# leeyevi/MV3D_TF

Measured on AMD Instinct MI355X. Metric: KITTI-shape frames/sec (RPN+3-view ROI-pool+NMS) at 1/2/4/8 MI355X, higher is better.
Workload: dtype f32

## Files before the change

include/mv3d_hip.h:

```cpp
#ifndef MV3D_HIP_H
#define MV3D_HIP_H
#include <stddef.h>
#include <stdint.h>
#ifdef __cplusplus
extern "C" {
#endif

typedef enum {
    MV3D_OK = 0,
    MV3D_ERR_INVALID_ARG = 1,
    MV3D_ERR_WORKSPACE = 2,
    MV3D_ERR_HIP = 3,
    MV3D_ERR_ZERO_DIVISION = 4
} mv3d_status;

int mv3d_version(void);
const char *mv3d_status_string(int status);


size_t mv3d_nms_workspace_bytes(int max_boxes);
int mv3d_nms_device(const float *dets_dev, int n, double thresh, int max_keep,
                    int32_t *keep_dev, int32_t *num_keep_dev, int32_t *status_dev,
                    void *workspace, size_t workspace_bytes, void *stream);

// ... 210 lines not shown
size_t mv3d_point_cloud_2_top_paper_workspace(int num_frames, const double *ranges8_host);
int mv3d_point_cloud_2_top_paper_shape(double res, double zres, double side_lo, double side_hi, double fwd_lo, double fwd_hi,
                                       double height_lo, double height_hi, int *dims);
int mv3d_bev_density_table(float *out64);

size_t mv3d_scan_crop_workspace(int total_points);
int mv3d_scan_crop_tile_rows(void);
int mv3d_scan_crop_to_image(const float *points_dev, const int32_t *offsets_dev, int num_frames, int total_points,
                            const float *calib_dev, const int32_t *image_hw_dev, float *points_out_dev, int32_t *offsets_out_dev,
                            void *workspace_dev, size_t workspace_bytes, void *stream);

int mv3d_scan_transform(const float *points_dev, const int32_t *offsets_dev, int num_frames, int total_points,
                        const double *xform_dev, float *points_out_dev, void *stream);

int mv3d_legacy_permutation(void *mt19937_state, int32_t n, int32_t *out);
typedef struct {
    int32_t n_fg, n_bg, n_low;
    int32_t pt_n_fg, pt_n_bg;
    int32_t reserved0;
    const uint8_t *fg_alive;
} mv3d_draw_frame;
typedef struct {
    int32_t rpn_batchsize;
    int32_t rpn_num_fg;
    int32_t rois_per_image;
    int32_t roi_fg_max;
} mv3d_draw_params;
int mv3d_draw_training_subsamples(void *mt19937_state, int batch, const mv3d_draw_frame *frames, const mv3d_draw_params *par,
                                  int32_t *lists, size_t lists_cap, int32_t *sizes, int32_t *scratch, size_t scratch_cap);

typedef struct {
    int32_t batch, H, W, num_classes;
    int32_t proposal_cap;
    int32_t anchor_cap;
    int32_t roi_cap;
    int32_t max_gt;
    mv3d_proposal_params proposal;
    mv3d_anchor_target_params anchor;
    mv3d_proposal_target_params target;
    mv3d_draw_params draw;
} mv3d_train_path_config;
typedef struct {
    float *blob_bv, *blob_img, *blob_3d;
    int32_t *num_proposals;
// ... 5 lines not shown
    int32_t *pt_counts;
    void *anchor_ws; size_t anchor_ws_bytes;
    void *target_ws; size_t target_ws_bytes;
    float *rois_bev, *rois_rgb, *rois_fv;
    float *rois_3d; int32_t *labels; float *bbox_targets;
    int32_t *lists; size_t lists_cap;
    uint8_t *h_report; size_t h_report_row;
    int32_t *h_pt_counts;
    int32_t *h_num_proposals;
    int32_t *h_lists;
    int32_t *h_scratch; size_t scratch_cap;
} mv3d_train_path_slot;
typedef struct mv3d_train_path mv3d_train_path;
int mv3d_train_path_create(const mv3d_train_path_config *config, int depth, const mv3d_train_path_slot *slots, int helper_thread,
                           mv3d_train_path **out);
int mv3d_train_path_configure(mv3d_train_path *path, const mv3d_train_path_config *config);
int mv3d_train_path_submit(mv3d_train_path *path, int slot, const float *prob_dev, const float *pred_dev, const float *im_info_dev,
                           const float *calib_dev, const float *const *gt_bv_dev, const float *const *gt_3d_dev,
                           const float *const *gt_corners_dev, const int *G, void *mt19937_state, void *stream);
int mv3d_train_path_submit_masked(mv3d_train_path *path, int slot, const float *prob_dev, const float *pred_dev,
                                  const float *im_info_dev, const float *calib_dev, const float *const *gt_bv_dev,
                                  const float *const *gt_3d_dev, const float *const *gt_corners_dev, const int *G,
                                  const uint8_t *anchor_mask_dev, void *mt19937_state, void *stream);
int mv3d_train_path_finish(mv3d_train_path *path, int slot, int32_t *rows_out, int32_t *num_proposals_out, int32_t *sizes_out);
int mv3d_train_path_host_seconds(mv3d_train_path *path, double *wait_s, double *draw_s);
void mv3d_train_path_destroy(mv3d_train_path *path);
int mv3d_train_path_launch_plan(const mv3d_train_path_config *config, int32_t *stage1_launches, int32_t *stage2_launches);

int mv3d_gt_encode(const float *box_cam_dev, const double *cos_sin_dev, int num_objects, const float *inv_rot_dev,
                   const float *tr_velo_to_cam_dev, float *corners_cam_dev, float *corners_lidar_dev,
                   float *boxes_3d_dev, float *boxes_bv_dev, void *stream);

int mv3d_box_detect_tail(const float *rois_3d_dev, const float *bbox_pred_dev, int num_rois, int num_classes,
                         float *corners_dev, float *pred_cnr_r_dev, float *pred_bv_dev, float *pred_bv_r_dev,
                         void *stream);

typedef struct {
    int32_t num_classes;
    int32_t rows_per_frame;
    int32_t max_per_image;
// ... 253 lines not shown
```

mv3d_tf_amd/_lib.py:

```python
import ctypes as C
import os

import torch

_HERE = os.path.dirname(os.path.abspath(__file__))
LIB_PATH = os.path.join(_HERE, "libmv3d_hip.so")

OK, ERR_INVALID_ARG, ERR_WORKSPACE, ERR_HIP, ERR_ZERO_DIVISION = 0, 1, 2, 3, 4
MAX_ROI_VIEWS = 4


class ProposalParams(C.Structure):
    _fields_ = [("feat_stride", C.c_int32), ("pre_nms_topN", C.c_int32), ("post_nms_topN", C.c_int32),
                ("img_height", C.c_int32), ("img_width", C.c_int32), ("img_padding", C.c_int32),
                ("nms_strict_gt", C.c_int32), ("reserved0", C.c_int32), ("nms_thresh", C.c_double), ("min_size", C.c_double)]


class DetectPostParams(C.Structure):
    _fields_ = [("num_classes", C.c_int32), ("rows_per_frame", C.c_int32), ("max_per_image", C.c_int32),
                ("nms_strict_gt", C.c_int32), ("score_thresh", C.c_float), ("reserved0", C.c_int32), ("nms_thresh", C.c_double)]


class AnchorTargetParams(C.Structure):
    _fields_ = [("feat_stride", C.c_int32), ("clobber_positives", C.c_int32),
# ... 189 lines not shown
    "mv3d_roi_pool_backward_workspace_bytes": (C.c_size_t, [C.c_int, C.POINTER(RoiGradView), C.c_int, C.c_int]),
    "mv3d_roi_pool_backward_views": (C.c_int, [C.c_int, C.POINTER(RoiGradView), C.c_int, C.c_int, _P, C.c_size_t, _P]),
    "mv3d_roi_pool_backward_path": (C.c_char_p, [C.c_int, C.POINTER(RoiGradView), C.c_int, C.c_int, C.c_int, C.c_int]),
    "mv3d_roi_pool_pair_workspace_bytes": (C.c_size_t, [C.c_int, C.POINTER(RoiGradView), C.c_int, C.c_int]),
    "mv3d_roi_pool_forward_views_pair": (C.c_int, [C.c_int, C.POINTER(RoiView), C.c_int, C.c_int, C.c_int, _P]),
    "mv3d_roi_pool_backward_views_pair": (C.c_int, [C.c_int, C.POINTER(RoiGradView), C.c_int, C.c_int, _P, C.c_size_t, _P]),
    "mv3d_roi_pool_argmax_decode": (C.c_int, [C.c_int, C.POINTER(RoiView), C.c_int, C.c_int, C.POINTER(C.c_void_p), _P]),
    "mv3d_ROIPoolForwardLaucher": (C.c_int, [_P, C.c_float, C.c_int, C.c_int, C.c_int, C.c_int, C.c_int, C.c_int, _P, _P, _P, _P]),
    "mv3d_ROIPoolBackwardLaucher": (C.c_int, [_P, C.c_float, C.c_int, C.c_int, C.c_int, C.c_int, C.c_int, C.c_int, C.c_int, _P, _P, _P, _P]),
    "mv3d_rois_3d_to_fv": (C.c_int, [_P, C.c_int, _P, _P]),
    "mv3d_point_cloud_2_front_workspace": (C.c_size_t, [C.c_int]),
    "mv3d_point_cloud_2_front": (C.c_int, [_P, _P, C.c_int, C.c_int, _P, _P, _P]),
    "mv3d_legacy_permutation": (C.c_int, [_P, C.c_int32, _P]),
    "mv3d_draw_training_subsamples": (C.c_int, [_P, C.c_int, C.POINTER(DrawFrame), C.POINTER(DrawParams), _P, C.c_size_t, _P, _P,
                                                C.c_size_t]),
    "mv3d_train_path_create": (C.c_int, [C.POINTER(TrainPathConfig), C.c_int, C.POINTER(TrainPathSlot), C.c_int, C.POINTER(C.c_void_p)]),
    "mv3d_train_path_configure": (C.c_int, [_P, C.POINTER(TrainPathConfig)]),
    "mv3d_train_path_submit": (C.c_int, [_P, C.c_int, _P, _P, _P, _P, _P, _P, _P, _P, _P, _P]),
    "mv3d_train_path_submit_masked": (C.c_int, [_P, C.c_int, _P, _P, _P, _P, _P, _P, _P, _P, _P, _P, _P]),
    "mv3d_train_path_finish": (C.c_int, [_P, C.c_int, _P, _P, _P]),
    "mv3d_train_path_host_seconds": (C.c_int, [_P, C.POINTER(C.c_double), C.POINTER(C.c_double)]),
    "mv3d_train_path_destroy": (None, [_P]),
    "mv3d_train_path_launch_plan": (C.c_int, [_P, C.POINTER(C.c_int32), C.POINTER(C.c_int32)]),
    "mv3d_gt_encode": (C.c_int, [_P, _P, C.c_int, _P, _P, _P, _P, _P, _P, _P]),
    "mv3d_conv3x3_f16": (C.c_int, [_P, _P, _P, _P, C.c_int, C.c_int, C.c_int, C.c_int, C.c_int, C.c_int, C.c_int, C.c_int, _P]),
    "mv3d_conv3x3_f32": (C.c_int, [_P, _P, _P, _P, C.c_int, C.c_int, C.c_int, C.c_int, C.c_int, C.c_int, C.c_int, _P]),
    "mv3d_maxpool2x2_f32": (C.c_int, [_P, _P, C.c_int, C.c_int, C.c_int, C.c_int, _P]),
    "mv3d_frame_nhwc_f32": (C.c_int, [_P, _P, C.c_int, C.c_int, C.c_int, C.c_int, C.c_int, _P]),
    "mv3d_conv3x3_bf16": (C.c_int, [_P, _P, _P, _P, C.c_int, C.c_int, C.c_int, C.c_int, C.c_int, C.c_int, C.c_int, C.c_int, _P]),
    "mv3d_maxpool2x2_bf16": (C.c_int, [_P, _P, C.c_int, C.c_int, C.c_int, C.c_int, _P]),
# ... 86 lines not shown
```

mv3d_tf_amd/csrc/legacy_rng.hip:

```cpp
#include <stdint.h>
#include <string.h>
#include "../../include/mv3d_hip.h"

namespace {

constexpr int MT_N = 624, MT_M = 397;
struct MtState { uint32_t key[MT_N]; int pos; };

inline void mt_gen(MtState *s)
{
    uint32_t *k = s->key;
    int i;
    for (i = 0; i < MT_N - MT_M; ++i) {
        const uint32_t y = (k[i] & 0x80000000u) | (k[i + 1] & 0x7fffffffu);
        k[i] = k[i + MT_M] ^ (y >> 1) ^ ((y & 1u) ? 0x9908b0dfu : 0u);
    }
    for (; i < MT_N - 1; ++i) {
        const uint32_t y = (k[i] & 0x80000000u) | (k[i + 1] & 0x7fffffffu);
        k[i] = k[i + (MT_M - MT_N)] ^ (y >> 1) ^ ((y & 1u) ? 0x9908b0dfu : 0u);
    }
    const uint32_t y = (k[MT_N - 1] & 0x80000000u) | (k[0] & 0x7fffffffu);
    k[MT_N - 1] = k[MT_M - 1] ^ (y >> 1) ^ ((y & 1u) ? 0x9908b0dfu : 0u);
    s->pos = 0;
}
// ... 33 lines not shown
                t_lo = pos;
            }
            while (pos < MT_N && i > lo) {
                const uint32_t j = t[pos++] & mask;
                const bool ok = j <= (uint32_t)i;
                const uint32_t jj = ok ? j : (uint32_t)i;
                const int32_t a = x[i], b = x[jj];
                x[i] = b; x[jj] = a;
                i -= ok ? 1 : 0;
            }
        }
    }
    s->pos = pos;
}

}

extern "C" int mv3d_legacy_permutation(void *mt19937_state, int32_t n, int32_t *out)
{
    if (!mt19937_state || n < 0 || (n > 0 && !out)) return MV3D_ERR_INVALID_ARG;
    MtState *s = (MtState *)mt19937_state;
    if (s->pos < 0 || s->pos > MT_N) return MV3D_ERR_INVALID_ARG;
    permutation(s, n, out);
    return MV3D_OK;
}

extern "C" int mv3d_draw_training_subsamples(void *mt19937_state, int batch, const mv3d_draw_frame *frames,
                                             const mv3d_draw_params *par, int32_t *lists, size_t lists_cap, int32_t *sizes,
                                             int32_t *scratch, size_t scratch_cap)
{
    if (!mt19937_state || batch <= 0 || !frames || !par || !lists || !sizes || !scratch) return MV3D_ERR_INVALID_ARG;
    MtState *s = (MtState *)mt19937_state;
    if (s->pos < 0 || s->pos > MT_N) return MV3D_ERR_INVALID_ARG;
    size_t o = 0;
    auto emit = [&](int32_t n, int32_t take, bool draw, int32_t *size_out) -> bool {
        *size_out = 0;
        if (!draw) return true;
        if (n < 0 || (size_t)n > scratch_cap || take < 0 || take > n || o + (size_t)take > lists_cap) return false;
        if (take == n) {
            permutation(s, n, lists + o);
        } else {
            permutation(s, n, scratch);
            memcpy(lists + o, scratch, (size_t)take * sizeof(int32_t));
        }
        *size_out = take;
        o += (size_t)take;
        return true;
    };
    for (int b = 0; b < batch; ++b) {
        const mv3d_draw_frame &f = frames[b];
        int32_t *sz = sizes + 5 * b;
        if (f.n_fg < 0 || f.n_bg < 0 || f.n_low < 0 || f.pt_n_fg < 0 || f.pt_n_bg < 0 || (f.n_fg > 0 && !f.fg_alive))
            return MV3D_ERR_INVALID_ARG;
        const int32_t num_fg = par->rpn_num_fg;
        const int32_t *dis_fg = lists + o;
        if (!emit(f.n_fg, f.n_fg - num_fg, f.n_fg > num_fg, &sz[0])) return MV3D_ERR_WORKSPACE;
        const int32_t num_bg = par->rpn_batchsize - (f.n_fg < num_fg ? f.n_fg : num_fg);
        if (!emit(f.n_bg, f.n_bg - num_bg, f.n_bg > num_bg, &sz[1])) return MV3D_ERR_WORKSPACE;
        int32_t n_pos = 0;
        if (f.n_fg > 0) {
            if ((size_t)f.n_fg > scratch_cap) return MV3D_ERR_WORKSPACE;
            uint8_t *alive = (uint8_t *)scratch;
            for (int32_t i = 0; i < f.n_fg; ++i) alive[i] = f.fg_alive[i] ? 1 : 0;
            for (int32_t i = 0; i < sz[0]; ++i) alive[dis_fg[i]] = 0;
            for (int32_t i = 0; i < f.n_fg; ++i) n_pos += alive[i];
        }
        const int32_t num_bg2 = par->rpn_batchsize - n_pos;
        if (!emit(f.n_low, f.n_low - num_bg2, f.n_low > num_bg2, &sz[2])) return MV3D_ERR_WORKSPACE;
        const int32_t fg_n = par->roi_fg_max < f.pt_n_fg ? par->roi_fg_max : f.pt_n_fg;
        if (!emit(f.pt_n_fg, fg_n, f.pt_n_fg > 0, &sz[3])) return MV3D_ERR_WORKSPACE;
        const int32_t bg_room = par->rois_per_image - fg_n;
        const int32_t bg_n = bg_room < f.pt_n_bg ? bg_room : f.pt_n_bg;
        if (!emit(f.pt_n_bg, bg_n < 0 ? 0 : bg_n, f.pt_n_bg > 0, &sz[4])) return MV3D_ERR_WORKSPACE;
    }
    return MV3D_OK;
}
```

mv3d_tf_amd/csrc/train_stream.hip:

```cpp
#include <hip/hip_runtime.h>
#include <chrono>
#include <condition_variable>
#include <deque>
#include <mutex>
#include <new>
#include <thread>
#include <vector>
#include "anchor_target.h"
#include "proposal.h"
#include "proposal_target.h"
#include "rank.h"

#define TP_MAX_BATCH 16

namespace {

enum SlotState { TP_IDLE = 0, TP_SUBMITTED = 1, TP_STAGED = 2 };

struct Slot {
    mv3d_train_path_slot buf;
    hipEvent_t ev = nullptr;
    int state = TP_IDLE, rc = MV3D_OK;
    hipStream_t stream = nullptr;
    void *mt = nullptr;
    const float *calib = nullptr;
    const float *gt_bv[TP_MAX_BATCH], *gt_3d[TP_MAX_BATCH], *gt_c[TP_MAX_BATCH];
    int G[TP_MAX_BATCH];
    int32_t sizes[5 * TP_MAX_BATCH], rows[TP_MAX_BATCH];
    std::vector<uint8_t> spill[TP_MAX_BATCH];
    float *p_bv[TP_MAX_BATCH], *p_3d[TP_MAX_BATCH];
    int32_t *p_num[TP_MAX_BATCH], *p_cnt[TP_MAX_BATCH], *a_cnt[TP_MAX_BATCH];
    uint8_t *a_fgh[TP_MAX_BATCH];
    void *a_ws[TP_MAX_BATCH], *p_ws[TP_MAX_BATCH];
    int p_cap[TP_MAX_BATCH];
    size_t p_wsz[TP_MAX_BATCH];
    uint8_t *dv_report = nullptr;
    int32_t *dv_pt_counts = nullptr, *dv_num_proposals = nullptr;
};

static bool tp_force_copies()
{
#ifdef MV3D_TUNING
    return getenv("MV3D_TRAIN_PATH_COPIES") != nullptr;
// ... 73 lines not shown
}

}

struct mv3d_train_path {
    mv3d_train_path_config cfg;
    mv3d_proposal_target_params tpar[TP_MAX_BATCH];
    int depth = 0, device = 0;
    std::vector<Slot> slots;
    bool threaded = false, stop = false;
    std::thread helper;
    std::mutex m;
    std::condition_variable cv_work, cv_done;
    std::deque<int> queue;
    double t_wait = 0.0, t_draw = 0.0;
    bool paired = false;
};

namespace {

bool config_ok(const mv3d_train_path_config &c)
{
    return c.batch >= 1 && c.batch <= TP_MAX_BATCH && c.H > 0 && c.W > 0 && c.num_classes >= 1 && c.proposal_cap > 0 && c.anchor_cap > 0 &&
           c.roi_cap > 0 && c.max_gt > 0 && c.draw.rois_per_image <= c.roi_cap;
}

void set_params(mv3d_train_path *tp, const mv3d_train_path_config &c)
{
    tp->cfg = c;
    TpPlan pl;
// ... 30 lines not shown
        s.p_cnt[b] = u.pt_counts + 4 * b;
        s.a_cnt[b] = (int32_t *)(u.report + (size_t)b * u.report_row);
        s.a_fgh[b] = u.report + (size_t)b * u.report_row + 32;
        s.a_ws[b] = (char *)u.anchor_ws + (size_t)b * u.anchor_ws_bytes;
        s.p_ws[b] = (char *)u.target_ws + (size_t)b * u.target_ws_bytes;
        s.p_cap[b] = c.proposal_cap;
        s.p_wsz[b] = u.target_ws_bytes;
    }
}

#define TP_HIP(expr)                                 \
    do {                                             \
        if ((expr) != hipSuccess) return MV3D_ERR_HIP; \
    } while (0)

int host_stage(mv3d_train_path *tp, Slot &s)
{
    const mv3d_train_path_config &c = tp->cfg;
    const mv3d_train_path_slot &u = s.buf;
    const int B = c.batch, H = c.H, W = c.W;
    const auto t0 = std::chrono::steady_clock::now();
    TP_HIP(hipEventSynchronize(s.ev));
    const auto t1 = std::chrono::steady_clock::now();
    for (int b = 0; b < B; ++b)
        if (u.h_num_proposals[B + b] & MV3D_FLAG_ZERO_DIVISION) return MV3D_ERR_ZERO_DIVISION;
    mv3d_draw_frame fr[TP_MAX_BATCH];
    for (int b = 0; b < B; ++b) {
        const uint8_t *head = u.h_report + (size_t)b * u.h_report_row;
        const int32_t *cnt = (const int32_t *)head;
        fr[b].n_fg = cnt[1]; fr[b].n_bg = cnt[2]; fr[b].n_low = cnt[3];
        fr[b].pt_n_fg = u.h_pt_counts[4 * b + 1]; fr[b].pt_n_bg = u.h_pt_counts[4 * b + 2];
        fr[b].reserved0 = 0;
        if (cnt[1] < 0 || (size_t)cnt[1] > (size_t)4 * H * W) return MV3D_ERR_INVALID_ARG;
        if (32 + (size_t)cnt[1] <= u.h_report_row) {
            fr[b].fg_alive = head + 32;
        } else {
            s.spill[b].resize((size_t)cnt[1]);
            TP_HIP(hipMemcpyAsync(s.spill[b].data(), s.a_fgh[b], (size_t)cnt[1], hipMemcpyDeviceToHost, s.stream));
            TP_HIP(hipStreamSynchronize(s.stream));
            fr[b].fg_alive = s.spill[b].data();
        }
    }
    int rc = mv3d_draw_training_subsamples(s.mt, B, fr, &c.draw, u.h_lists, u.lists_cap, s.sizes, u.h_scratch, u.scratch_cap);
    const auto t2 = std::chrono::steady_clock::now();
    {
        std::lock_guard<std::mutex> g(tp->m);
        tp->t_wait += std::chrono::duration<double>(t1 - t0).count();
        tp->t_draw += std::chrono::duration<double>(t2 - t1).count();
    }
    if (rc != MV3D_OK) return rc;
    size_t off[5 * TP_MAX_BATCH + 1];
    off[0] = 0;
    for (int k = 0; k < 5 * B; ++k) off[k + 1] = off[k] + (size_t)s.sizes[k];
    const int32_t *const lists = u.lists;
    if (off[5 * B]) TP_HIP(hipMemcpyAsync(u.lists, u.h_lists, off[5 * B] * sizeof(int32_t), hipMemcpyHostToDevice, s.stream));
    const int32_t *lst[5][TP_MAX_BATCH];
    int cnt[5][TP_MAX_BATCH];
    for (int b = 0; b < B; ++b)
        for (int k = 0; k < 5; ++k) {
            cnt[k][b] = s.sizes[5 * b + k];
            lst[k][b] = cnt[k][b] ? lists + off[5 * b + k] : nullptr;
        }
    float *o_bev[TP_MAX_BATCH], *o_rgb[TP_MAX_BATCH], *o_fv[TP_MAX_BATCH], *o_3d[TP_MAX_BATCH], *o_tg[TP_MAX_BATCH];
    int32_t *o_lab[TP_MAX_BATCH];
    const float *cal[TP_MAX_BATCH];
// ... 25 lines not shown
    int most_dis, most_rois;
    rc = at_stage2_args(B, H, W, &c.anchor, lst[0], cnt[0], lst[1], cnt[1], lst[2], cnt[2], u.rpn_labels, u.anchors, u.anchors_3d, u.n_anchors,
                        c.anchor_cap, s.a_ws, u.anchor_ws_bytes, at, L, most_dis);
    if (rc != MV3D_OK) return rc;
    rc = pt_stage2_args(B, s.p_bv, s.p_3d, s.p_cap, s.p_num, s.gt_bv, s.gt_3d, s.gt_c, s.G, cal, tp->tpar, lst[3], cnt[3], lst[4], cnt[4], o_bev,
                        o_rgb, o_lab, o_tg, o_3d, u.rois_fv ? o_fv : nullptr, s.p_ws, s.p_wsz, pt, most_rois);
    if (rc != MV3D_OK) return rc;
    TpStage2 a;
    for (int b = 0; b < TP_MAX_BATCH; ++b) { a.at[b] = at_emit_frame(at.f[b]); a.pt[b] = pt_emit_frame(pt.f[b]); }
    a.g = at_emit_grid(at.f[0], at.cap);
    if (most_dis > 0) hipLaunchKernelGGL(tp_disable_all_kernel, dim3((most_dis + 255) / 256, B), dim3(256), 0, s.stream, at);
    hipLaunchKernelGGL(tp_stage2_kernel, dim3(L.ncwg + pt_emit_workgroups(most_rois), B), dim3(256), 0, s.stream, a, L.ncwg);
    return mv3d_launch_status();
}

int host_stage_noexcept(mv3d_train_path *tp, Slot &s)
{
    try {
        return host_stage(tp, s);
    } catch (...) {
        return MV3D_ERR_WORKSPACE;
    }
}

int stage1_single(mv3d_train_path *tp, Slot &s, const float *prob, const float *pred, const float *im_info, const uint8_t *anchor_mask,
                  const uint8_t *const *masks)
{
    const mv3d_train_path_config &c = tp->cfg;
    const mv3d_train_path_slot &u = s.buf;
    const int B = c.batch;
    int rc = mv3d_proposal_3d_masked(prob, pred, B, c.H, c.W, im_info, s.calib, &c.proposal, anchor_mask, u.blob_bv, u.blob_img, u.blob_3d,
                                     u.num_proposals, u.num_proposals + B, u.proposal_ws, u.proposal_ws_bytes, s.stream);
    if (rc != MV3D_OK) return rc;
    rc = mv3d_anchor_target_stage1_batch_masked(B, c.H, c.W, im_info, s.gt_bv, s.gt_3d, s.G, &c.anchor, masks, u.rpn_labels, u.rpn_targets,
                                                s.a_cnt, s.a_fgh, s.a_ws, u.anchor_ws_bytes, s.stream);
    if (rc != MV3D_OK) return rc;
    rc = mv3d_proposal_target_stage1_batch_devn(B, s.p_bv, s.p_3d, s.p_cap, s.p_num, s.gt_bv, s.gt_3d, s.G, tp->tpar, s.p_cnt, s.p_ws,
// ... 37 lines not shown
    hipLaunchKernelGGL(tp_rank_label_kernel, dim3(AL.nblk + n_rank, B), dim3(RANK_NSUB * RANK_LK), 0, s.stream, a, r, AL.nblk, n_rank);
    hipLaunchKernelGGL(tp_merge_compact_kernel, dim3(AL.ncwg + n_rank, B), dim3(256), 0, s.stream, a, r, AL.ncwg);
    if (mv3d_launch_status() != MV3D_OK) return MV3D_ERR_HIP;
    rc = mv3d_launch_nms(nl, s.stream);
    if (rc != MV3D_OK) return rc;
    PtMirror mirror = {};
    mirror.batch = B;
    if (s.dv_report) {
        mirror.report = u.report; mirror.h_report = s.dv_report; mirror.report_row = u.report_row; mirror.h_row = u.h_report_row;
        mirror.h_pt_counts = s.dv_pt_counts; mirror.num_proposals = u.num_proposals; mirror.h_num_proposals = s.dv_num_proposals;
    }
    return mv3d_pt_stage1_batch_mirrored(B, s.p_bv, s.p_3d, s.p_cap, s.p_num, s.gt_bv, s.gt_3d, s.G, tp->tpar, s.p_cnt, s.p_ws, s.p_wsz, mirror,
                                         s.stream);
}

void helper_main(mv3d_train_path *tp)
{
    (void)hipSetDevice(tp->device);
    for (;;) {
        int k;
        {
            std::unique_lock<std::mutex> g(tp->m);
            tp->cv_work.wait(g, [&] { return tp->stop || !tp->queue.empty(); });
            if (tp->queue.empty()) return;
            k = tp->queue.front();
            tp->queue.pop_front();
        }
        Slot &s = tp->slots[k];
        const int rc = host_stage_noexcept(tp, s);
        {
            std::lock_guard<std::mutex> g(tp->m);
            s.rc = rc;
            s.state = TP_STAGED;
        }
        tp->cv_done.notify_all();
    }
}

}

extern "C" int mv3d_train_path_create(const mv3d_train_path_config *config, int depth, const mv3d_train_path_slot *slots, int helper_thread,
                                      mv3d_train_path **out)
{
    if (!config || !slots || !out || depth < 1 || depth > 64 || !config_ok(*config)) return MV3D_ERR_INVALID_ARG;
    for (int k = 0; k < depth; ++k)
        if (!slot_ok(*config, slots[k])) return MV3D_ERR_INVALID_ARG;
    mv3d_train_path *tp = new (std::nothrow) mv3d_train_path();
    if (!tp) return MV3D_ERR_HIP;
    set_params(tp, *config);
    tp->depth = depth;
    if (hipGetDevice(&tp->device) != hipSuccess) { delete tp; return MV3D_ERR_HIP; }
    try {
        tp->slots.resize((size_t)depth);
    } catch (...) {
        delete tp;
        return MV3D_ERR_HIP;
    }
    for (int k = 0; k < depth; ++k) {
        Slot &s = tp->slots[k];
// ... 5 lines not shown
                                hipHostGetDevicePointer(&d2, s.buf.h_num_proposals, 0) == hipSuccess && d0 && d1 && d2;
            (void)hipGetLastError();
            if (mapped && s.buf.h_report_row % 16 == 0 && (uintptr_t)d0 % 16 == 0 && (uintptr_t)s.buf.report % 16 == 0 && !tp_force_copies()) {
                s.dv_report = (uint8_t *)d0; s.dv_pt_counts = (int32_t *)d1; s.dv_num_proposals = (int32_t *)d2;
            }
        }
        if (hipEventCreateWithFlags(&s.ev, hipEventDisableTiming | hipEventBlockingSync) != hipSuccess) {
            for (int j = 0; j < k; ++j) (void)hipEventDestroy(tp->slots[j].ev);
            delete tp;
            return MV3D_ERR_HIP;
        }
    }
    tp->threaded = helper_thread != 0;
    if (tp->threaded) {
        try {
            tp->helper = std::thread(helper_main, tp);
        } catch (...) {
            for (Slot &s : tp->slots) (void)hipEventDestroy(s.ev);
            delete tp;
            return MV3D_ERR_HIP;
        }
    }
    *out = tp;
    return MV3D_OK;
}

extern "C" int mv3d_train_path_configure(mv3d_train_path *tp, const mv3d_train_path_config *c)
{
    if (!tp || !c || !config_ok(*c)) return MV3D_ERR_INVALID_ARG;
    const mv3d_train_path_config &o = tp->cfg;
    if (c->batch != o.batch || c->H != o.H || c->W != o.W || c->num_classes != o.num_classes || c->proposal_cap != o.proposal_cap ||
        c->anchor_cap != o.anchor_cap || c->roi_cap != o.roi_cap || c->max_gt != o.max_gt)
// ... 87 lines not shown
    std::lock_guard<std::mutex> g(tp->m);
    s.state = TP_IDLE;
    return rc;
}

extern "C" int mv3d_train_path_host_seconds(mv3d_train_path *tp, double *wait_s, double *draw_s)
{
    if (!tp) return MV3D_ERR_INVALID_ARG;
    std::lock_guard<std::mutex> g(tp->m);
    if (wait_s) *wait_s = tp->t_wait;
    if (draw_s) *draw_s = tp->t_draw;
    tp->t_wait = tp->t_draw = 0.0;
    return MV3D_OK;
}

extern "C" int mv3d_train_path_launch_plan(const mv3d_train_path_config *c, int32_t *stage1, int32_t *stage2)
{
    TpPlan pl;
    if (!c || !config_ok(*c) || !tp_plan(*c, pl)) return -1;
    if (stage1) *stage1 = pl.stage1;
    if (stage2) *stage2 = pl.stage2;
    return pl.paired ? 1 : 0;
}

extern "C" void mv3d_train_path_destroy(mv3d_train_path *tp)
{
    if (!tp) return;
    if (tp->threaded) {
        {
            std::lock_guard<std::mutex> g(tp->m);
            tp->stop = true;
        }
        tp->cv_work.notify_all();
        tp->helper.join();
    }
    for (Slot &s : tp->slots)
        if (s.ev) (void)hipEventDestroy(s.ev);
    delete tp;
}
```

mv3d_tf_amd/train_path.py:

```python
import ctypes as C

import numpy as np
import torch

from . import ops
from ._lib import DrawParams, TrainPathConfig, TrainPathSlot, check, lib
from .fast_rcnn.config import cfg
from .rpn_msr.anchor_target_layer_tf import REPORT_HEAD as _HEAD

def _global_mt19937_address():
    bg = np.random.mtrand._rand._bit_generator
    if not isinstance(bg, np.random.MT19937):
        raise TypeError("TrainPathStream draws on numpy's global legacy MT19937; the global bit generator is a %s" % type(bg).__name__)
    return bg.ctypes.state_address


class _Slot:
    pass


class TrainPathStream:

    def __init__(self, B, H, W, device, num_classes=2, depth=2, max_gt=64, want_fv=True, stream=None, async_draws=True, streams=None):
        self.B, self.H, self.W, self.dev, self.nc = int(B), int(H), int(W), torch.device(device), int(num_classes)
        self.N = self.H * self.W * 4
        self.want_fv = bool(want_fv)
        self.stream = stream
        self.streams = list(streams) if streams else None
        self.max_gt = int(max_gt)
        T = cfg.TRAIN
        self.anchor_cap = ops.anchor_debug_rows(T)
        self.roi_cap = int(T.BATCH_SIZE)
        L = lib()
        self.pparams = ops.proposal_params(T)
        self.cap = L.mv3d_proposal_3d_capacity(self.H, self.W, C.byref(self.pparams))
        if self.cap < 0:
            check(1, "mv3d_proposal_3d_capacity")
        self._cfg_key, self._config = self._make_config()
        self.slots = [self._make_slot(k) for k in range(int(depth))]
        for k, sl_ in enumerate(self.slots):
            sl_.stream = self.streams[k % len(self.streams)] if self.streams else self.stream
        self._slots_c = (TrainPathSlot * len(self.slots))(*[sl_.c for sl_ in self.slots])
        self._h = C.c_void_p()
        self.async_draws = bool(async_draws)
        with torch.cuda.device(self.dev):
            check(L.mv3d_train_path_create(C.byref(self._config), len(self.slots), self._slots_c, 1 if self.async_draws else 0,
                                           C.byref(self._h)), "mv3d_train_path_create")
        self._next = 0

    def _make_config(self):
        T = cfg.TRAIN
        rois_per_image = int(T.BATCH_SIZE) // 1
        key = (float(T.FG_THRESH), float(T.BG_THRESH_HI), float(T.BG_THRESH_LO), int(T.RPN_BATCHSIZE), float(T.RPN_FG_FRACTION),
               float(T.FG_FRACTION), rois_per_image, bool(T.RPN_CLOBBER_POSITIVES), float(T.RPN_NEGATIVE_OVERLAP), float(T.RPN_POSITIVE_OVERLAP))
        c = TrainPathConfig()
        c.batch, c.H, c.W, c.num_classes = self.B, self.H, self.W, self.nc
        c.proposal_cap, c.anchor_cap, c.roi_cap, c.max_gt = self.cap, self.anchor_cap, self.roi_cap, self.max_gt
        c.proposal = self.pparams
        c.anchor = ops.anchor_target_params(T)
        c.target = ops.proposal_target_params(T, self.nc)
        c.draw = DrawParams(int(T.RPN_BATCHSIZE), int(T.RPN_FG_FRACTION * T.RPN_BATCHSIZE), rois_per_image,
                            int(np.round(T.FG_FRACTION * rois_per_image)))
# ... 84 lines not shown
        if h:
            lib().mv3d_train_path_destroy(h)

    def __del__(self):
        try:
            self.close()
        except Exception:
            pass

    @property
    def host_seconds(self):
        w, d = C.c_double(), C.c_double()
        check(lib().mv3d_train_path_host_seconds(self._h, C.byref(w), C.byref(d)), "mv3d_train_path_host_seconds")
        return w.value, d.value

    def finish(self, s):
        s.busy = False
        check(lib().mv3d_train_path_finish(self._h, s.index, s.rows_c, s.nprop_c, s.sizes_c), "mv3d_train_path_finish")
        S = list(s.rows_c)
        St = sum(S)
        return {"rpn_labels": s.rpn_labels, "rpn_targets": s.rpn_targets, "anchors": s.anchors, "anchors_3d": s.anchors_3d,
                "n_anchors": s.n_anchors, "rois": {k: v[:St] for k, v in s.rois.items()}, "rois_3d": s.rois_3d[:St],
                "labels": s.labels[:St], "bbox_targets": s.bbox_targets[:St], "S": S,
                "num_proposals": list(s.nprop_c), "proposals": s.prop, "stream": s.stream, "draw_sizes": list(s.sizes_c)}
```

Before: 17200.

## Parallelize large legacy-RNG permutation draws across worker threads via state snapshots

Large background-sample permutations in the host-side training subsample draw are now deferred. The helper thread snapshots the MT19937 state and advances it with a fast skip-ahead routine (batched rejection counting, AVX2 variant) that does not materialize the permutation. Worker threads then replay the snapshotted permutations in parallel, and the last worker runs the tail stage. The aim is to take serial host RNG work off the training pipeline's critical path. The cost is extra threads, synchronization, and complexity around keeping the RNG stream bit-exact.

```diff
diff --git a/include/mv3d_hip.h b/include/mv3d_hip.h
--- a/include/mv3d_hip.h
+++ b/include/mv3d_hip.h
@@ -248,6 +248,7 @@
                         const double *xform_dev, float *points_out_dev, void *stream);
 
 int mv3d_legacy_permutation(void *mt19937_state, int32_t n, int32_t *out);
+int mv3d_legacy_permutation_advance(void *mt19937_state, int32_t n, int force_portable);
 typedef struct {
     int32_t n_fg, n_bg, n_low;
     int32_t pt_n_fg, pt_n_bg;
@@ -262,6 +263,9 @@
 } mv3d_draw_params;
 int mv3d_draw_training_subsamples(void *mt19937_state, int batch, const mv3d_draw_frame *frames, const mv3d_draw_params *par,
                                   int32_t *lists, size_t lists_cap, int32_t *sizes, int32_t *scratch, size_t scratch_cap);
+int mv3d_draw_training_subsamples_mt(void *mt19937_state, int batch, const mv3d_draw_frame *frames, const mv3d_draw_params *par,
+                                     int32_t *lists, size_t lists_cap, int32_t *sizes, int32_t *scratch, size_t scratch_cap,
+                                     int workers);
 
 typedef struct {
     int32_t batch, H, W, num_classes;
@@ -297,6 +301,8 @@
 typedef struct mv3d_train_path mv3d_train_path;
 int mv3d_train_path_create(const mv3d_train_path_config *config, int depth, const mv3d_train_path_slot *slots, int helper_thread,
                            mv3d_train_path **out);
+int mv3d_train_path_create_ex(const mv3d_train_path_config *config, int depth, const mv3d_train_path_slot *slots, int helper_thread,
+                              int draw_workers, mv3d_train_path **out);
 int mv3d_train_path_configure(mv3d_train_path *path, const mv3d_train_path_config *config);
 int mv3d_train_path_submit(mv3d_train_path *path, int slot, const float *prob_dev, const float *pred_dev, const float *im_info_dev,
                            const float *calib_dev, const float *const *gt_bv_dev, const float *const *gt_3d_dev,
@@ -307,6 +313,7 @@
                                   const uint8_t *anchor_mask_dev, void *mt19937_state, void *stream);
 int mv3d_train_path_finish(mv3d_train_path *path, int slot, int32_t *rows_out, int32_t *num_proposals_out, int32_t *sizes_out);
 int mv3d_train_path_host_seconds(mv3d_train_path *path, double *wait_s, double *draw_s);
+int mv3d_train_path_host_profile(mv3d_train_path *path, double out[8]);
 void mv3d_train_path_destroy(mv3d_train_path *path);
 int mv3d_train_path_launch_plan(const mv3d_train_path_config *config, int32_t *stage1_launches, int32_t *stage2_launches);
 
diff --git a/mv3d_tf_amd/_lib.py b/mv3d_tf_amd/_lib.py
--- a/mv3d_tf_amd/_lib.py
+++ b/mv3d_tf_amd/_lib.py
@@ -227,6 +227,12 @@
     "mv3d_legacy_permutation": (C.c_int, [_P, C.c_int32, _P]),
     "mv3d_draw_training_subsamples": (C.c_int, [_P, C.c_int, C.POINTER(DrawFrame), C.POINTER(DrawParams), _P, C.c_size_t, _P, _P,
                                                 C.c_size_t]),
+    "mv3d_legacy_permutation_advance": (C.c_int, [_P, C.c_int32, C.c_int]),
+    "mv3d_draw_training_subsamples_mt": (C.c_int, [_P, C.c_int, C.POINTER(DrawFrame), C.POINTER(DrawParams), _P, C.c_size_t, _P, _P,
+                                                   C.c_size_t, C.c_int]),
+    "mv3d_train_path_create_ex": (C.c_int, [C.POINTER(TrainPathConfig), C.c_int, C.POINTER(TrainPathSlot), C.c_int, C.c_int,
+                                            C.POINTER(C.c_void_p)]),
+    "mv3d_train_path_host_profile": (C.c_int, [_P, C.POINTER(C.c_double)]),
     "mv3d_train_path_create": (C.c_int, [C.POINTER(TrainPathConfig), C.c_int, C.POINTER(TrainPathSlot), C.c_int, C.POINTER(C.c_void_p)]),
     "mv3d_train_path_configure": (C.c_int, [_P, C.POINTER(TrainPathConfig)]),
     "mv3d_train_path_submit": (C.c_int, [_P, C.c_int, _P, _P, _P, _P, _P, _P, _P, _P, _P, _P]),
diff --git a/mv3d_tf_amd/csrc/legacy_rng.h b/mv3d_tf_amd/csrc/legacy_rng.h
--- /dev/null
+++ b/mv3d_tf_amd/csrc/legacy_rng.h
@@ -0,0 +1,20 @@
+#pragma once
+#include <stddef.h>
+#include <stdint.h>
+#include "../../include/mv3d_hip.h"
+
+#define MV3D_MT_N 624
+struct Mv3dMtState { uint32_t key[MV3D_MT_N]; int pos; };
+
+#define MV3D_DRAW_DEFER_MIN 4096
+
+struct Mv3dDrawJob {
+    Mv3dMtState snapshot;
+    int32_t n, take;
+    int32_t *dst;
+};
+
+int mv3d_draw_plan(void *mt19937_state, int batch, const mv3d_draw_frame *frames, const mv3d_draw_params *par, int32_t *lists,
+                   size_t lists_cap, int32_t *sizes, int32_t *scratch, size_t scratch_cap, int32_t defer_min, Mv3dDrawJob *jobs,
+                   int max_jobs, int *njobs);
+void mv3d_draw_replay(const Mv3dDrawJob *job, int32_t *scratch);
diff --git a/mv3d_tf_amd/csrc/legacy_rng.hip b/mv3d_tf_amd/csrc/legacy_rng.hip
--- a/mv3d_tf_amd/csrc/legacy_rng.hip
+++ b/mv3d_tf_amd/csrc/legacy_rng.hip
@@ -1,13 +1,18 @@
 #include <stdint.h>
 #include <string.h>
-#include "../../include/mv3d_hip.h"
+#include <atomic>
+#include <thread>
+#include <vector>
+#include "legacy_rng.h"
 
 namespace {
 
-constexpr int MT_N = 624, MT_M = 397;
-struct MtState { uint32_t key[MT_N]; int pos; };
-
-inline void mt_gen(MtState *s)
+constexpr int MT_N = MV3D_MT_N, MT_M = 397;
+using MtState = Mv3dMtState;
+
+#define MT_INLINE inline __attribute__((always_inline))
+
+MT_INLINE void mt_gen(MtState *s)
 {
     uint32_t *k = s->key;
     int i;
@@ -71,6 +76,65 @@
     s->pos = pos;
 }
 
+constexpr int ADV_W = 32;
+MT_INLINE void advance_body(MtState *s, int32_t n)
+{
+    int32_t i = n - 1;
+    int pos = s->pos;
+    uint32_t t[MT_N];
+    int t_lo = MT_N;
+    while (i >= 1) {
+        const uint32_t mask = 0xffffffffu >> __builtin_clz((uint32_t)i);
+        const int32_t lo = (int32_t)(mask >> 1);
+        while (i > lo) {
+            if (pos == MT_N) { mt_gen(s); pos = 0; t_lo = MT_N; }
+            if (t_lo > pos) {
+                for (int k = pos; k < MT_N; ++k) {
+                    uint32_t y = s->key[k];
+                    y ^= (y >> 11);
+                    y ^= (y << 7) & 0x9d2c5680u;
+                    y ^= (y << 15) & 0xefc60000u;
+                    y ^= (y >> 18);
+                    t[k] = y;
+                }
+                t_lo = pos;
+            }
+            while (pos + ADV_W <= MT_N && i - ADV_W > lo) {
+                const int32_t sure = i - ADV_W;
+                int below = 0, within = 0;
+                for (int k = 0; k < ADV_W; ++k) {
+                    const int32_t v = (int32_t)(t[pos + k] & mask);
+                    below += v <= sure ? 1 : 0;
+                    within += v <= i ? 1 : 0;
+                }
+                if (below != within) {
+                    below = 0;
+                    for (int k = 0; k < ADV_W; ++k) below += (int32_t)(t[pos + k] & mask) <= i - below ? 1 : 0;
+                }
+                i -= below;
+                pos += ADV_W;
+            }
+            while (pos < MT_N && i > lo) i -= (t[pos++] & mask) <= (uint32_t)i ? 1 : 0;
+        }
+    }
+    s->pos = pos;
+}
+
+void advance_portable(MtState *s, int32_t n) { advance_body(s, n); }
+#if defined(__x86_64__) && !defined(__HIP_DEVICE_COMPILE__)
+#define MV3D_ADVANCE_AVX2 1
+__attribute__((target("avx2"))) void advance_avx2(MtState *s, int32_t n) { advance_body(s, n); }
+#endif
+
+void advance_permutation(MtState *s, int32_t n, bool force_portable = false)
+{
+#ifdef MV3D_ADVANCE_AVX2
+    static const bool wide = __builtin_cpu_supports("avx2");
+    if (wide && !force_portable) { advance_avx2(s, n); return; }
+#endif
+    advance_portable(s, n);
+}
+
 }
 
 extern "C" int mv3d_legacy_permutation(void *mt19937_state, int32_t n, int32_t *out)
@@ -82,20 +146,37 @@
     return MV3D_OK;
 }
 
-extern "C" int mv3d_draw_training_subsamples(void *mt19937_state, int batch, const mv3d_draw_frame *frames,
-                                             const mv3d_draw_params *par, int32_t *lists, size_t lists_cap, int32_t *sizes,
-                                             int32_t *scratch, size_t scratch_cap)
-{
+extern "C" int mv3d_legacy_permutation_advance(void *mt19937_state, int32_t n, int force_portable)
+{
+    if (!mt19937_state || n < 0) return MV3D_ERR_INVALID_ARG;
+    MtState *s = (MtState *)mt19937_state;
+    if (s->pos < 0 || s->pos > MT_N) return MV3D_ERR_INVALID_ARG;
+    advance_permutation(s, n, force_portable != 0);
+    return MV3D_OK;
+}
+
+int mv3d_draw_plan(void *mt19937_state, int batch, const mv3d_draw_frame *frames, const mv3d_draw_params *par, int32_t *lists,
+                   size_t lists_cap, int32_t *sizes, int32_t *scratch, size_t scratch_cap, int32_t defer_min, Mv3dDrawJob *jobs,
+                   int max_jobs, int *njobs)
+{
+    if (njobs) *njobs = 0;
     if (!mt19937_state || batch <= 0 || !frames || !par || !lists || !sizes || !scratch) return MV3D_ERR_INVALID_ARG;
+    if (defer_min > 0 && (!jobs || !njobs || max_jobs < 2 * batch)) return MV3D_ERR_INVALID_ARG;
     MtState *s = (MtState *)mt19937_state;
     if (s->pos < 0 || s->pos > MT_N) return MV3D_ERR_INVALID_ARG;
     size_t o = 0;
-    auto emit = [&](int32_t n, int32_t take, bool draw, int32_t *size_out) -> bool {
+    int nj = 0;
+    auto emit = [&](int32_t n, int32_t take, bool draw, int32_t *size_out, bool big) -> bool {
         *size_out = 0;
         if (!draw) return true;
         if (n < 0 || (size_t)n > scratch_cap || take < 0 || take > n || o + (size_t)take > lists_cap) return false;
         if (take == n) {
             permutation(s, n, lists + o);
+        } else if (big && defer_min > 0 && n >= defer_min) {
+            Mv3dDrawJob &j = jobs[nj++];
+            j.snapshot = *s;
+            j.n = n; j.take = take; j.dst = lists + o;
+            advance_permutation(s, n);
         } else {
             permutation(s, n, scratch);
             memcpy(lists + o, scratch, (size_t)take * sizeof(int32_t));
@@ -111,9 +192,9 @@
             return MV3D_ERR_INVALID_ARG;
         const int32_t num_fg = par->rpn_num_fg;
         const int32_t *dis_fg = lists + o;
-        if (!emit(f.n_fg, f.n_fg - num_fg, f.n_fg > num_fg, &sz[0])) return MV3D_ERR_WORKSPACE;
+        if (!emit(f.n_fg, f.n_fg - num_fg, f.n_fg > num_fg, &sz[0], false)) return MV3D_ERR_WORKSPACE;
         const int32_t num_bg = par->rpn_batchsize - (f.n_fg < num_fg ? f.n_fg : num_fg);
-        if (!emit(f.n_bg, f.n_bg - num_bg, f.n_bg > num_bg, &sz[1])) return MV3D_ERR_WORKSPACE;
+        if (!emit(f.n_bg, f.n_bg - num_bg, f.n_bg > num_bg, &sz[1], true)) return MV3D_ERR_WORKSPACE;
         int32_t n_pos = 0;
         if (f.n_fg > 0) {
             if ((size_t)f.n_fg > scratch_cap) return MV3D_ERR_WORKSPACE;
@@ -123,12 +204,63 @@
             for (int32_t i = 0; i < f.n_fg; ++i) n_pos += alive[i];
         }
         const int32_t num_bg2 = par->rpn_batchsize - n_pos;
-        if (!emit(f.n_low, f.n_low - num_bg2, f.n_low > num_bg2, &sz[2])) return MV3D_ERR_WORKSPACE;
+        if (!emit(f.n_low, f.n_low - num_bg2, f.n_low > num_bg2, &sz[2], true)) return MV3D_ERR_WORKSPACE;
         const int32_t fg_n = par->roi_fg_max < f.pt_n_fg ? par->roi_fg_max : f.pt_n_fg;
-        if (!emit(f.pt_n_fg, fg_n, f.pt_n_fg > 0, &sz[3])) return MV3D_ERR_WORKSPACE;
+        if (!emit(f.pt_n_fg, fg_n, f.pt_n_fg > 0, &sz[3], false)) return MV3D_ERR_WORKSPACE;
         const int32_t bg_room = par->rois_per_image - fg_n;
         const int32_t bg_n = bg_room < f.pt_n_bg ? bg_room : f.pt_n_bg;
-        if (!emit(f.pt_n_bg, bg_n < 0 ? 0 : bg_n, f.pt_n_bg > 0, &sz[4])) return MV3D_ERR_WORKSPACE;
-    }
+        if (!emit(f.pt_n_bg, bg_n < 0 ? 0 : bg_n, f.pt_n_bg > 0, &sz[4], false)) return MV3D_ERR_WORKSPACE;
+    }
+    if (njobs) *njobs = nj;
     return MV3D_OK;
 }
+
+void mv3d_draw_replay(const Mv3dDrawJob *job, int32_t *scratch)
+{
+    MtState s = job->snapshot;
+    permutation(&s, job->n, scratch);
+    memcpy(job->dst, scratch, (size_t)job->take * sizeof(int32_t));
+}
+
+extern "C" int mv3d_draw_training_subsamples(void *mt19937_state, int batch, const mv3d_draw_frame *frames,
+                                             const mv3d_draw_params *par, int32_t *lists, size_t lists_cap, int32_t *sizes,
+                                             int32_t *scratch, size_t scratch_cap)
+{
+    return mv3d_draw_plan(mt19937_state, batch, frames, par, lists, lists_cap, sizes, scratch, scratch_cap, 0, nullptr, 0, nullptr);
+}
+
+extern "C" int mv3d_draw_training_subsamples_mt(void *mt19937_state, int batch, const mv3d_draw_frame *frames,
+                                                const mv3d_draw_params *par, int32_t *lists, size_t lists_cap, int32_t *sizes,
+                                                int32_t *scratch, size_t scratch_cap, int workers)
+{
+    if (workers < 0 || workers > 64) return MV3D_ERR_INVALID_ARG;
+    if (workers == 0 || batch <= 0)
+        return mv3d_draw_plan(mt19937_state, batch, frames, par, lists, lists_cap, sizes, scratch, scratch_cap, 0, nullptr, 0, nullptr);
+    try {
+        std::vector<Mv3dDrawJob> jobs((size_t)2 * batch);
+        int nj = 0;
+        const int rc = mv3d_draw_plan(mt19937_state, batch, frames, par, lists, lists_cap, sizes, scratch, scratch_cap, MV3D_DRAW_DEFER_MIN,
+                                      jobs.data(), 2 * batch, &nj);
+        if (rc != MV3D_OK || nj == 0) return rc;
+        int32_t most = 0;
+        for (int j = 0; j < nj; ++j) most = jobs[j].n > most ? jobs[j].n : most;
+        const int nt = workers < nj ? workers : nj;
+        std::vector<std::vector<int32_t>> own((size_t)nt);
+        for (auto &v : own) v.resize((size_t)most);
+        std::atomic<int> next(0);
+        std::vector<std::thread> pool;
+        pool.reserve((size_t)nt);
+        auto work = [&](int w) {
+            for (int j = next.fetch_add(1); j < nj; j = next.fetch_add(1)) mv3d_draw_replay(&jobs[j], own[w].data());
+        };
+        try {
+            for (int w = 0; w < nt; ++w) pool.emplace_back(work, w);
+        } catch (...) {
+            if (pool.empty()) work(0);
+        }
+        for (std::thread &t : pool) t.join();
+        return MV3D_OK;
+    } catch (...) {
+        return MV3D_ERR_WORKSPACE;
+    }
+}
diff --git a/mv3d_tf_amd/csrc/train_stream.hip b/mv3d_tf_amd/csrc/train_stream.hip
--- a/mv3d_tf_amd/csrc/train_stream.hip
+++ b/mv3d_tf_amd/csrc/train_stream.hip
@@ -1,4 +1,6 @@
 #include <hip/hip_runtime.h>
+#include <sched.h>
+#include <stdlib.h>
 #include <chrono>
 #include <condition_variable>
 #include <deque>
@@ -7,6 +9,7 @@
 #include <thread>
 #include <vector>
 #include "anchor_target.h"
+#include "legacy_rng.h"
 #include "proposal.h"
 #include "proposal_target.h"
 #include "rank.h"
@@ -27,6 +30,8 @@
     const float *gt_bv[TP_MAX_BATCH], *gt_3d[TP_MAX_BATCH], *gt_c[TP_MAX_BATCH];
     int G[TP_MAX_BATCH];
     int32_t sizes[5 * TP_MAX_BATCH], rows[TP_MAX_BATCH];
+    std::vector<Mv3dDrawJob> jobs;
+    int njobs = 0, pending = 0;
     std::vector<uint8_t> spill[TP_MAX_BATCH];
     float *p_bv[TP_MAX_BATCH], *p_3d[TP_MAX_BATCH];
     int32_t *p_num[TP_MAX_BATCH], *p_cnt[TP_MAX_BATCH], *a_cnt[TP_MAX_BATCH];
@@ -130,6 +135,13 @@
     std::condition_variable cv_work, cv_done;
     std::deque<int> queue;
     double t_wait = 0.0, t_draw = 0.0;
+    int n_workers = 0;
+    bool wstop = false;
+    std::vector<std::thread> workers;
+    std::vector<std::vector<int32_t>> wscratch;
+    std::condition_variable cv_jobs;
+    std::deque<std::pair<int, int>> jobq;
+    double prof[8] = {0, 0, 0, 0, 0, 0, 0, 0};
     bool paired = false;
 };
 
@@ -190,11 +202,17 @@
         if ((expr) != hipSuccess) return MV3D_ERR_HIP; \
     } while (0)
 
-int host_stage(mv3d_train_path *tp, Slot &s)
+inline double tp_seconds(std::chrono::steady_clock::time_point a, std::chrono::steady_clock::time_point b)
+{
+    return std::chrono::duration<double>(b - a).count();
+}
+
+int host_plan(mv3d_train_path *tp, Slot &s, bool defer)
 {
     const mv3d_train_path_config &c = tp->cfg;
     const mv3d_train_path_slot &u = s.buf;
     const int B = c.batch, H = c.H, W = c.W;
+    s.njobs = 0;
     const auto t0 = std::chrono::steady_clock::now();
     TP_HIP(hipEventSynchronize(s.ev));
     const auto t1 = std::chrono::steady_clock::now();
@@ -217,14 +235,27 @@
             fr[b].fg_alive = s.spill[b].data();
         }
     }
-    int rc = mv3d_draw_training_subsamples(s.mt, B, fr, &c.draw, u.h_lists, u.lists_cap, s.sizes, u.h_scratch, u.scratch_cap);
+    defer = defer && s.jobs.size() >= (size_t)2 * B;
+    const int rc = mv3d_draw_plan(s.mt, B, fr, &c.draw, u.h_lists, u.lists_cap, s.sizes, u.h_scratch, u.scratch_cap,
+                                  defer ? MV3D_DRAW_DEFER_MIN : 0, defer ? s.jobs.data() : nullptr, defer ? (int)s.jobs.size() : 0, &s.njobs);
     const auto t2 = std::chrono::steady_clock::now();
     {
         std::lock_guard<std::mutex> g(tp->m);
-        tp->t_wait += std::chrono::duration<double>(t1 - t0).count();
-        tp->t_draw += std::chrono::duration<double>(t2 - t1).count();
-    }
-    if (rc != MV3D_OK) return rc;
+        tp->t_wait += tp_seconds(t0, t1);
+        tp->t_draw += tp_seconds(t1, t2);
+        tp->prof[0] += tp_seconds(t0, t1);
+        tp->prof[1] += tp_seconds(t1, t2);
+        tp->prof[6] += 1.0;
+    }
+    return rc;
+}
+
+int host_tail(mv3d_train_path *tp, Slot &s)
+{
+    const mv3d_train_path_config &c = tp->cfg;
+    const mv3d_train_path_slot &u = s.buf;
+    const int B = c.batch, H = c.H, W = c.W;
+    int rc;
     size_t off[5 * TP_MAX_BATCH + 1];
     off[0] = 0;
     for (int k = 0; k < 5 * B; ++k) off[k + 1] = off[k] + (size_t)s.sizes[k];
@@ -280,13 +311,29 @@
     return mv3d_launch_status();
 }
 
-int host_stage_noexcept(mv3d_train_path *tp, Slot &s)
+int host_plan_noexcept(mv3d_train_path *tp, Slot &s, bool defer)
 {
     try {
-        return host_stage(tp, s);
+        return host_plan(tp, s, defer);
     } catch (...) {
         return MV3D_ERR_WORKSPACE;
     }
+}
+
+int host_tail_timed(mv3d_train_path *tp, Slot &s)
+{
+    const auto t0 = std::chrono::steady_clock::now();
+    const int rc = host_tail(tp, s);
+    const auto t1 = std::chrono::steady_clock::now();
+    std::lock_guard<std::mutex> g(tp->m);
+    tp->prof[4] += tp_seconds(t0, t1);
+    return rc;
+}
+
+int host_stage_noexcept(mv3d_train_path *tp, Slot &s)
+{
+    const int rc = host_plan_noexcept(tp, s, false);
+    return rc != MV3D_OK ? rc : host_tail_timed(tp, s);
 }
 
 int stage1_single(mv3d_train_path *tp, Slot &s, const float *prob, const float *pred, const float *im_info, const uint8_t *anchor_mask,
@@ -354,27 +401,124 @@
                                          s.stream);
 }
 
+void slot_staged(mv3d_train_path *tp, Slot &s, int rc)
+{
+    {
+        std::lock_guard<std::mutex> g(tp->m);
+        s.rc = rc;
+        s.state = TP_STAGED;
+    }
+    tp->cv_done.notify_all();
+}
+
 void helper_main(mv3d_train_path *tp)
 {
     (void)hipSetDevice(tp->device);
+    const bool defer = tp->n_workers > 0;
     for (;;) {
         int k;
         {
             std::unique_lock<std::mutex> g(tp->m);
+            const auto t0 = std::chrono::steady_clock::now();
             tp->cv_work.wait(g, [&] { return tp->stop || !tp->queue.empty(); });
+            tp->prof[2] += tp_seconds(t0, std::chrono::steady_clock::now());
             if (tp->queue.empty()) return;
             k = tp->queue.front();
             tp->queue.pop_front();
         }
         Slot &s = tp->slots[k];
-        const int rc = host_stage_noexcept(tp, s);
+        int rc = host_plan_noexcept(tp, s, defer);
+        if (rc == MV3D_OK && s.njobs > 0) {
+            bool queued = true;
+            {
+                std::lock_guard<std::mutex> g(tp->m);
+                int j = 0;
+                try {
+                    for (; j < s.njobs; ++j) tp->jobq.emplace_back(k, j);
+                } catch (...) {
+                    for (; j > 0; --j) tp->jobq.pop_back();
+                    queued = false;
+                }
+                if (queued) s.pending = s.njobs;
+            }
+            if (queued) {
+                tp->cv_jobs.notify_all();
+                continue;
+            }
+            for (int j = 0; j < s.njobs; ++j) mv3d_draw_replay(&s.jobs[j], s.buf.h_scratch);
+        }
+        if (rc == MV3D_OK) rc = host_tail_timed(tp, s);
+        slot_staged(tp, s, rc);
+    }
+}
+
+void worker_main(mv3d_train_path *tp, int w)
+{
+    (void)hipSetDevice(tp->device);
+    int32_t *scratch = tp->wscratch[(size_t)w].data();
+    for (;;) {
+        std::pair<int, int> job;
+        {
+            std::unique_lock<std::mutex> g(tp->m);
+            const auto t0 = std::chrono::steady_clock::now();
+            tp->cv_jobs.wait(g, [&] { return tp->wstop || !tp->jobq.empty(); });
+            tp->prof[5] += tp_seconds(t0, std::chrono::steady_clock::now());
+            if (tp->jobq.empty()) return;
+            job = tp->jobq.front();
+            tp->jobq.pop_front();
+        }
+        Slot &s = tp->slots[job.first];
+        const auto t0 = std::chrono::steady_clock::now();
+        mv3d_draw_replay(&s.jobs[job.second], scratch);
+        const auto t1 = std::chrono::steady_clock::now();
+        bool last;
         {
             std::lock_guard<std::mutex> g(tp->m);
-            s.rc = rc;
-            s.state = TP_STAGED;
-        }
-        tp->cv_done.notify_all();
-    }
+            tp->prof[3] += tp_seconds(t0, t1);
+            tp->prof[7] += 1.0;
+            last = --s.pending == 0;
+        }
+        if (last) slot_staged(tp, s, host_tail_timed(tp, s));
+    }
+}
+
+int default_draw_workers()
+{
+    const char *e = getenv("MV3D_DRAW_WORKERS");
+    if (e && *e) {
+        char *end = nullptr;
+        const long v = strtol(e, &end, 10);
+        if (end != e && *end == 0 && v >= 0 && v <= 4) return (int)v;
+    }
+    int n = 0;
+    const int max_cpus = 8192;
+    cpu_set_t *set = CPU_ALLOC(max_cpus);
+    if (set) {
+        const size_t sz = CPU_ALLOC_SIZE(max_cpus);
+        CPU_ZERO_S(sz, set);
+        if (sched_getaffinity(0, sz, set) == 0) n = CPU_COUNT_S(sz, set);
+        CPU_FREE(set);
+    }
+    return n - 2 < 0 ? 0 : (n - 2 > 2 ? 2 : n - 2);
+}
+
+void join_threads(mv3d_train_path *tp)
+{
+    if (tp->helper.joinable()) {
+        {
+            std::lock_guard<std::mutex> g(tp->m);
+            tp->stop = true;
+        }
+        tp->cv_work.notify_all();
+        tp->helper.join();
+    }
+    {
+        std::lock_guard<std::mutex> g(tp->m);
+        tp->wstop = true;
+    }
+    tp->cv_jobs.notify_all();
+    for (std::thread &t : tp->workers)
+        if (t.joinable()) t.join();
 }
 
 }
@@ -382,7 +526,14 @@
 extern "C" int mv3d_train_path_create(const mv3d_train_path_config *config, int depth, const mv3d_train_path_slot *slots, int helper_thread,
                                       mv3d_train_path **out)
 {
-    if (!config || !slots || !out || depth < 1 || depth > 64 || !config_ok(*config)) return MV3D_ERR_INVALID_ARG;
+    return mv3d_train_path_create_ex(config, depth, slots, helper_thread, -1, out);
+}
+
+extern "C" int mv3d_train_path_create_ex(const mv3d_train_path_config *config, int depth, const mv3d_train_path_slot *slots, int helper_thread,
+                                         int draw_workers, mv3d_train_path **out)
+{
+    if (!config || !slots || !out || depth < 1 || depth > 64 || !config_ok(*config) || draw_workers < -1 || draw_workers > 4)
+        return MV3D_ERR_INVALID_ARG;
     for (int k = 0; k < depth; ++k)
         if (!slot_ok(*config, slots[k])) return MV3D_ERR_INVALID_ARG;
     mv3d_train_path *tp = new (std::nothrow) mv3d_train_path();
@@ -418,8 +569,21 @@
     tp->threaded = helper_thread != 0;
     if (tp->threaded) {
         try {
+            tp->n_workers = draw_workers < 0 ? default_draw_workers() : draw_workers;
+            if (tp->n_workers > 0) {
+                size_t most = 0;
+                for (Slot &s : tp->slots) {
+                    s.jobs.resize((size_t)2 * config->batch);
+                    most = s.buf.scratch_cap > most ? s.buf.scratch_cap : most;
+                }
+                tp->wscratch.resize((size_t)tp->n_workers);
+                for (auto &v : tp->wscratch) v.resize(most);
+                tp->workers.reserve((size_t)tp->n_workers);
+                for (int w = 0; w < tp->n_workers; ++w) tp->workers.emplace_back(worker_main, tp, w);
+            }
             tp->helper = std::thread(helper_main, tp);
         } catch (...) {
+            join_threads(tp);
             for (Slot &s : tp->slots) (void)hipEventDestroy(s.ev);
             delete tp;
             return MV3D_ERR_HIP;
@@ -537,6 +701,14 @@
     return MV3D_OK;
 }
 
+extern "C" int mv3d_train_path_host_profile(mv3d_train_path *tp, double out[8])
+{
+    if (!tp || !out) return MV3D_ERR_INVALID_ARG;
+    std::lock_guard<std::mutex> g(tp->m);
+    for (int i = 0; i < 8; ++i) { out[i] = tp->prof[i]; tp->prof[i] = 0.0; }
+    return MV3D_OK;
+}
+
 extern "C" int mv3d_train_path_launch_plan(const mv3d_train_path_config *c, int32_t *stage1, int32_t *stage2)
 {
     TpPlan pl;
@@ -549,14 +721,7 @@
 extern "C" void mv3d_train_path_destroy(mv3d_train_path *tp)
 {
     if (!tp) return;
-    if (tp->threaded) {
-        {
-            std::lock_guard<std::mutex> g(tp->m);
-            tp->stop = true;
-        }
-        tp->cv_work.notify_all();
-        tp->helper.join();
-    }
+    join_threads(tp);
     for (Slot &s : tp->slots)
         if (s.ev) (void)hipEventDestroy(s.ev);
     delete tp;
diff --git a/mv3d_tf_amd/train_path.py b/mv3d_tf_amd/train_path.py
--- a/mv3d_tf_amd/train_path.py
+++ b/mv3d_tf_amd/train_path.py
@@ -21,7 +21,8 @@
 
 class TrainPathStream:
 
-    def __init__(self, B, H, W, device, num_classes=2, depth=2, max_gt=64, want_fv=True, stream=None, async_draws=True, streams=None):
+    def __init__(self, B, H, W, device, num_classes=2, depth=2, max_gt=64, want_fv=True, stream=None, async_draws=True, streams=None,
+                 draw_workers=None):
         self.B, self.H, self.W, self.dev, self.nc = int(B), int(H), int(W), torch.device(device), int(num_classes)
         self.N = self.H * self.W * 4
         self.want_fv = bool(want_fv)
@@ -44,8 +45,9 @@
         self._h = C.c_void_p()
         self.async_draws = bool(async_draws)
         with torch.cuda.device(self.dev):
-            check(L.mv3d_train_path_create(C.byref(self._config), len(self.slots), self._slots_c, 1 if self.async_draws else 0,
-                                           C.byref(self._h)), "mv3d_train_path_create")
+            check(L.mv3d_train_path_create_ex(C.byref(self._config), len(self.slots), self._slots_c, 1 if self.async_draws else 0,
+                                              -1 if draw_workers is None else int(draw_workers), C.byref(self._h)),
+                  "mv3d_train_path_create_ex")
         self._next = 0
 
     def _make_config(self):
@@ -160,6 +162,13 @@
         check(lib().mv3d_train_path_host_seconds(self._h, C.byref(w), C.byref(d)), "mv3d_train_path_host_seconds")
         return w.value, d.value
 
+    @property
+    def host_profile(self):
+        out = (C.c_double * 8)()
+        check(lib().mv3d_train_path_host_profile(self._h, out), "mv3d_train_path_host_profile")
+        keys = ("helper_wait_s", "helper_plan_s", "helper_idle_s", "worker_replay_s", "enqueue_s", "worker_idle_s", "batches", "replays")
+        return dict(zip(keys, out))
+
     def finish(self, s):
         s.busy = False
         check(lib().mv3d_train_path_finish(self._h, s.index, s.rows_c, s.nprop_c, s.sizes_c), "mv3d_train_path_finish")
```

Measured after the change: 16740. -2.7%, worse.
